# Gyeeta/gyeeta

Hardware: AMD Instinct MI355X
Metric: events/sec ingested + p50/p99 quantile error vs reference, 1→8 MI355X (higher is better)
Workload: dtype int64; 1 GPU; C3/C4: 10000 hosts x 1000 services, raw 24-B tcp_ipv4_resp_event_t stream, uniform over services, 1 window (ingest + window close) per step; service_keys_total=10000000, multi_level_windows=0, td_pend_cap=1920, td_pend_cap_is_library_default=False, exchange=none, exchange_requested=none, exchange_fallback=False

## Files before the change

### gyeeta_amd/csrc/gys_device.hpp

```cpp
#pragma once

#include <hip/hip_runtime.h>
#include <stdint.h>

#include "../../include/gysketch.h"
#include "../../include/gys_tdigest_tbl.h"

#define GYS_WAVE 64
#ifndef GYS_OPAQUE_VGPR
#define GYS_OPAQUE_VGPR(x) asm volatile("" : "+v"(x))
#endif
#ifndef GYS_DYN_LDS
#define GYS_DYN_LDS(type, name) extern __shared__ type name[]
#endif
#define GYS_SEED 0xceedfeadu
#define GYS_GOLDEN 0x9e3779b9u
#define GYS_NOSLOT 0xFFFFFFFFu
#define GYS_EMPTY_KEY 0xFFFFFFFFFFFFFFFFull

#ifndef GYS_KERNARG
#define GYS_KERNARG 1
#endif
#if GYS_KERNARG && defined(__HIP_DEVICE_COMPILE__)
#define GYS_KERNARG_REF(T, name, arg)                                                             \
// ... 61 lines not shown
	jmix(a, b, c);
	return c;
}

__host__ __device__ __forceinline__ uint32_t jhash2_4w(uint32_t k0, uint32_t k1, uint32_t k2, uint32_t k3, uint32_t initval)
{
	uint32_t a = GYS_GOLDEN + k0, b = GYS_GOLDEN + k1, c = initval + k2;
	jmix(a, b, c);
	c += 16u;
	a += k3;
	jmix(a, b, c);
	return c;
}

__host__ __device__ __forceinline__ uint32_t jhash2_u64(uint64_t key, uint32_t initval)
{
	uint32_t a = GYS_GOLDEN, b = GYS_GOLDEN, c = initval;
	c += 8;
	b += (uint32_t)(key >> 32);
	a += (uint32_t)(key & 0xFFFFFFFFu);
	jmix(a, b, c);
	return c;
}

__host__ __device__ __forceinline__ uint32_t host_tbl_hash(uint32_t netns, uint32_t port)
{
	uint32_t x = netns ^ ((port & 0xFFFFu) * 0x9E3779u);
	x ^= x >> 16;
	return x * 0x85EBCA6Bu;
}
__host__ __device__ __forceinline__ uint32_t host_tbl_hash(uint64_t key48) { return host_tbl_hash((uint32_t)(key48 >> 16), (uint32_t)(key48 & 0xFFFFu)); }
__host__ __device__ __forceinline__ uint32_t host_tbl_slot(uint32_t hk, uint32_t mask) { return (hk ^ (hk >> 13)) & mask; }
__host__ __device__ __forceinline__ uint32_t host_tbl_part(uint32_t hk, uint32_t pmask) { return (hk >> 21) & pmask; }

struct HashDef {
	int32_t nthr;
	int32_t is_fixed_diff;
	int32_t arg_bits, t_bits;
	int64_t thr[14];
	int64_t fd_min, fd_maxp1, fd_diff;
};

#define GYS_HASH_DEFS_INIT                                                                                                  \
	{                                                                                                                   \
		{13, 0, 64, 64, {1, 10, 30, 60, 100, 150, 200, 300, 450, 700, 1000, 3000, 15000}, 0, 0, 0},                      \
		{12, 0, 32, 32, {1, 10, 100, 500, 1000, 5000, 25000, 50000, 100000, 300000, 1000000, 5000000}, 0, 0, 0},      \
		{13, 0, 32, 32, {1, 10, 50, 200, 500, 1000, 3000, 6000, 10000, 15000, 25000, 60000, 150000}, 0, 0, 0},        \
		{13, 0, 32, 32, {1, 10, 25, 50, 125, 400, 1000, 3000, 6000, 10000, 25000, 40000, 65000}, 0, 0, 0},            \
		{12, 0, 32, 32, {10, 25, 50, 75, 100, 150, 300, 500, 800, 1000, 2000, 5000}, 0, 0, 0},                          \
		{10, 0, 32, 32, {5, 10, 20, 40, 60, 80, 100, 140, 200, 250}, 0, 0, 0},                                          \
		{12, 0, 32, 32, {1, 5, 10, 25, 50, 75, 100, 150, 300, 500, 1000, 3000}, 0, 0, 0},                               \
		{11, 1, 64, 32, {9, 19, 29, 39, 49, 59, 69, 79, 89, 99, 100}, 0, 101, 10},                                      \
	}

__constant__ HashDef d_hash_defs[GYS_NUM_HASH_KINDS] = GYS_HASH_DEFS_INIT;
static const HashDef h_hash_defs[GYS_NUM_HASH_KINDS] = GYS_HASH_DEFS_INIT;

__host__ __device__ inline const HashDef &hash_def(int kind)
{
#ifdef __HIP_DEVICE_COMPILE__
	return d_hash_defs[kind];
#else
	return h_hash_defs[kind];
#endif
}

// ... 286 lines not shown
```

### gyeeta_amd/csrc/gys_engine.hip

```cpp
#include <hip/hip_runtime.h>

#include <algorithm>
#include <array>
#include <atomic>
#include <chrono>
#include <cmath>
#include <cstdarg>
#include <cstdio>
#include <cstdlib>
#include <cstring>
#include <deque>
#include <map>
#include <string>
#include <thread>
#include <condition_variable>
#include <mutex>
#include <unordered_map>
#include <unordered_set>
#include <vector>

#include <dlfcn.h>
#include <rccl/rccl.h>

#include "gys_kernels.hpp"
// ... 31 lines not shown
struct MachIdHash {
	size_t operator()(const MachId &m) const
	{
		uint32_t w[4];
		memcpy(w, &m.first, 8);
		memcpy(w + 2, &m.second, 8);
		uint32_t k[6] = {w[0], w[1], w[2], w[3], 0, 0};
		return jhash2<6>(k, 4, GYS_SEED);
	}
};

inline MachId to_machid(const uint8_t id[16])
{
	MachId m;
	memcpy(&m.first, id, 8);
	memcpy(&m.second, id + 8, 8);
	return m;
}

struct ProfEntry {
	double total_ms = 0;
	uint64_t launches = 0;
	std::vector<std::pair<hipEvent_t, hipEvent_t>> pending;
};

inline uint64_t align_up(uint64_t v, uint64_t a) { return (v + a - 1) / a * a; }

struct HostListeners {
	std::vector<uint64_t> tbl;
	std::vector<uint32_t> slots;
	std::vector<uint32_t> all_slots;
	std::vector<uint64_t> keys;
	uint32_t tbl_off = 0, tbl_cap = 0, lst_off = 0;
	bool on_device = false;
	bool overflow = false;
	std::vector<HostListeners> sub;
	uint32_t sub_desc = 0;
	struct LAddr {
		uint32_t ip32 = 0;
		uint32_t ip128[4] = {0, 0, 0, 0};
		bool any = true;
	};
	struct ChainEnt {
		uint32_t slot;
		LAddr a;
	};
	std::unordered_map<uint64_t, std::vector<ChainEnt>> chain;
	std::vector<ListenerCand> cands;
	std::unordered_map<uint64_t, uint32_t> cand_first;
	uint32_t cand_off = 0, cand_cap = 0;
	bool dirty = false;
	std::unordered_map<uint64_t, uint32_t> okey;
};

#define GYS_HOST_MAX_LOCAL 2048u
#define GYS_HOST_MAX_PARTS 16u

struct ArenaLayout {
	uint64_t off_hll8, off_u32, n_u32, off_i64sum, n_i64sum, off_i64max, n_i64max, total;
	uint64_t u32_cms, u32_cluster, u32_pair, u32_misc, u32_cpair;
	uint64_t i64_cms, i64_ghist, i64_pair, i64_cpair;
};

ArenaLayout arena_layout(uint32_t max_clusters, bool conn_pair)
{
	ArenaLayout a;
// ... 414 lines not shown
void host_tbl_put(HostListeners &hl, uint64_t key48, uint32_t local)
{
	const uint32_t mask = (uint32_t)hl.tbl.size() - 1;
	uint32_t h = host_tbl_slot(host_tbl_hash(key48), mask);
	while (hl.tbl[h] != GYS_HOST_TBL_EMPTY) h = (h + 1) & mask;
	hl.tbl[h] = (key48 << 16) | (uint64_t)local;
}

inline uint32_t host_part_of(uint64_t key48, uint32_t nparts) { return host_tbl_part(host_tbl_hash(key48), nparts - 1u); }

#define GYS_HOST_TBL_SPARSE 4096u
inline uint32_t host_tbl_capacity(size_t n)
{
	static const uint32_t sparse = [] { const char *e = getenv("GYS_TBL_SPARSE"); return e ? (uint32_t)atoi(e) : GYS_HOST_TBL_SPARSE; }();
	const uint32_t c4 = next_pow2(std::max<uint64_t>(16, (uint64_t)n * 4));
	return c4 <= sparse ? c4 : std::max<uint32_t>(std::min<uint32_t>(sparse, c4), next_pow2(std::max<uint64_t>(16, (uint64_t)n * 2)));
}

int host_tbl_upload(gys_ctx *c, HostListeners &hl, uint32_t desc, uint32_t part, uint32_t nparts, uint32_t cand_off, bool *ok)
{
	*ok = true;
	if (!hl.on_device || hl.tbl.size() > hl.tbl_cap) {
		if (c->htbl_used + hl.tbl.size() > c->htbl_cap || c->hlst_used + hl.tbl.size() / 2 > c->hlst_cap) {
			*ok = false;
			return GYS_OK;
		}
		hl.tbl_off = (uint32_t)c->htbl_used;
		hl.tbl_cap = (uint32_t)hl.tbl.size();
		c->htbl_used += hl.tbl.size();
		hl.lst_off = (uint32_t)c->hlst_used;
		c->hlst_used += hl.tbl.size() / 2;
		hl.on_device = true;
	}
	HIPCHK(hipMemcpyAsync(c->htbl + hl.tbl_off, hl.tbl.data(), hl.tbl.size() * 8, hipMemcpyHostToDevice, c->stream));
	if (!hl.slots.empty()) HIPCHK(hipMemcpyAsync(c->hlst + hl.lst_off, hl.slots.data(), hl.slots.size() * 4, hipMemcpyHostToDevice, c->stream));
	const HostDesc hd{hl.tbl_off, (uint32_t)hl.tbl.size() - 1, (uint32_t)hl.slots.size(), hl.lst_off, part, nparts - 1u, cand_off, 0u};
	HIPCHK(hipMemcpyAsync(c->hdesc + desc, &hd, sizeof(hd), hipMemcpyHostToDevice, c->stream));
	HIPCHK(hipStreamSynchronize(c->stream));
	return GYS_OK;
}

int host_cands_upload(gys_ctx *c, HostListeners &hl)
{
	if (hl.cands.empty()) return GYS_OK;
	if (hl.cands.size() > hl.cand_cap) {
		const uint64_t want = std::max<uint64_t>(16, next_pow2(hl.cands.size()));
		const uint64_t bound = 4ull * c->cfg.max_services + 64ull * c->cfg.max_hosts;
		if (c->cand_used + want > bound) {
			set_err("listener candidate pool exhausted");
			return GYS_ERR_NOMEM;
		}
		if (c->cand_used + want > c->cand_cap) {
			uint64_t ncap = std::max<uint64_t>(c->cand_cap * 2, 4096);
			while (ncap < c->cand_used + want) ncap *= 2;
			ncap = std::min(ncap, bound);
			ListenerCand *np = nullptr;
			HIPCHK(hipMalloc((void **)&np, ncap * sizeof(ListenerCand)));
			if (c->cand_pool) {
				HIPCHK(hipMemcpyAsync(np, c->cand_pool, c->cand_used * sizeof(ListenerCand), hipMemcpyDeviceToDevice, c->stream));
				HIPCHK(hipStreamSynchronize(c->stream));
				HIPCHK(hipFree(c->cand_pool));
			}
			c->cand_pool = np;
			c->cand_cap = ncap;
		}
		hl.cand_off = (uint32_t)c->cand_used;
		hl.cand_cap = (uint32_t)want;
		c->cand_used += want;
	}
// ... 325 lines not shown
	const bool td = c->cfg.enable_tdigest != 0;
	if (td && n > c->cfg.max_batch_events) {
		set_err("batch of %llu events exceeds max_batch_events %llu", (unsigned long long)n, (unsigned long long)c->cfg.max_batch_events);
		return GYS_ERR_NOMEM;
	}
	if (n >= (1ull << 31)) {
		set_err("batch too large (u32 offsets)");
		return GYS_ERR_INVAL;
	}
	for (uint32_t s = 0; s < nsegs; ++s) {
		if (segs_host[s].host_slot >= c->hosts.size() || segs_host[s].first_event > n || (s && segs_host[s].first_event < segs_host[s - 1].first_event)) {
			set_err("bad resp segment %u", s);
			return GYS_ERR_INVAL;
		}
	}
	gys_ctx::SegSlot &slot = c->seg_ring[c->seg_next];
	c->seg_next = (c->seg_next + 1) % GYS_SEG_RING;
	if (!slot.done) HIPCHK(hipEventCreateWithFlags(&slot.done, hipEventDisableTiming));
	HIPCHK(hipEventSynchronize(slot.done));
	if (nsegs > slot.cap) {
		if (slot.host) HIPCHK(hipHostFree(slot.host));
		if (slot.dev) HIPCHK(hipFree(slot.dev));
		slot.host = slot.dev = nullptr;
		slot.cap = std::max<uint32_t>(nsegs, 1024);
		HIPCHK(hipHostMalloc((void **)&slot.host, (uint64_t)slot.cap * sizeof(gys_resp_seg), hipHostMallocDefault));
		HIPCHK(hipMalloc((void **)&slot.dev, (uint64_t)slot.cap * sizeof(gys_resp_seg)));
	}
	memcpy(slot.host, segs_host, (uint64_t)nsegs * sizeof(gys_resp_seg));
	for (uint32_t s = 0; s < nsegs; ++s) ((gys_resp_seg *)slot.host)[s].reserved = 0;
	HIPCHK(hipMemcpyAsync(slot.dev, slot.host, (uint64_t)nsegs * sizeof(gys_resp_seg), hipMemcpyHostToDevice, c->stream));
	const gys_resp_seg *segs_dev = slot.dev;

	bool host_local = td && c->cfg.resp_path != 1 && c->nsvc != 0, host_split = false, host_parts = false;
	uint32_t max_tbl = 16, max_l = 1;
	uint64_t max_len = 0, nwg = 0;
	bool cands = false;
	if (host_local) {
		c->batch_stamp++;
		for (uint32_t s = 0; s < nsegs && host_local; ++s) {
			const uint32_t host = segs_host[s].host_slot;
			const HostListeners &hl = c->host_lst[host];
			cands = cands || !hl.chain.empty();
			const uint64_t len = (s + 1 < nsegs ? segs_host[s + 1].first_event : n) - segs_host[s].first_event;
			if (c->host_seen[host] == c->batch_stamp || hl.overflow) host_local = false;
			c->host_seen[host] = c->batch_stamp;
			max_len = std::max(max_len, len);
			if (hl.sub.empty()) {
				if (!hl.on_device) host_local = false;
				max_tbl = std::max<uint32_t>(max_tbl, (uint32_t)hl.tbl.size());
				max_l = std::max<uint32_t>(max_l, (uint32_t)hl.slots.size());
				nwg += 1;
			} else {
				host_parts = true;
				for (const HostListeners &t : hl.sub) {
					if (!t.on_device) host_local = false;
					max_tbl = std::max<uint32_t>(max_tbl, (uint32_t)t.tbl.size());
					max_l = std::max<uint32_t>(max_l, (uint32_t)t.slots.size());
				}
				nwg += hl.sub.size();
			}
		}
		const double t_host = (double)((nwg + c->ncu - 1) / c->ncu) * (double)max_len / 0.35e9;
		const double t_split = (double)n * (double)std::max<uint64_t>(nwg, 1) / (double)std::max<uint32_t>(nsegs, 1) / 40.0e9 + 20e-6;
		if (host_local && max_len > GYS_SPLIT_PART && (c->cfg.resp_path == 3 || (c->cfg.resp_path == 0 && t_split < t_host))) host_split = true;
	}
	const int mode = v6 ? 2 : cands ? 1 : 0;
	const uint32_t nsvc = c->nsvc;
	uint32_t *cms32 = (uint32_t *)(c->arena + c->al.off_u32) + c->al.u32_cms;
	unsigned long long *ghist = (unsigned long long *)(c->arena + c->al.off_i64sum) + c->al.i64_ghist;
	long long *gmax = (long long *)(c->arena + c->al.off_i64max);
	if (td) {
		HIPCHK(hipMemsetAsync(c->merge_count, 0, 8 * 4, c->stream));
		c->resp_dirty = true;
	}
	FinP fin{};
	if (td) {
		fin.td_cur = c->td_cur;
		fin.td_meta = c->td_meta;
		fin.nsvc = c->nsvc;
		fin.pcap = c->pcap;
		fin.pend_cap = c->pend_cap;
		fin.merge_fast = c->merge_fast;
		static const bool class2_huge = getenv("GYS_CLASS2_HUGE") != nullptr || getenv("GYS_OLD_HUGE") != nullptr;
		fin.class2_max = class2_huge ? 0u : GYS_MERGE_LDS_MAX;
		fin.epoch = c->epoch;
		fin.resp_win = c->resp_win;
		fin.list[FIN_CLASS0] = c->merge_list;
		fin.list[FIN_CLASS1] = c->merge_list1;
		fin.list[FIN_CLASS2] = c->merge_list2;
// ... 67 lines not shown
			if (xbytes > slot.xcap) {
				if (slot.xhost) HIPCHK(hipHostFree(slot.xhost));
				if (slot.xdev) HIPCHK(hipFree(slot.xdev));
				slot.xhost = slot.xdev = nullptr;
				slot.xcap = std::max<uint64_t>(xbytes, 1u << 16);
				HIPCHK(hipHostMalloc((void **)&slot.xhost, slot.xcap, hipHostMallocDefault));
				HIPCHK(hipMalloc((void **)&slot.xdev, slot.xcap));
			}
			gys_resp_seg *vseg = (gys_resp_seg *)slot.xhost;
			uint64_t v = 0;
			for (uint32_t s = 0; s < nsegs; ++s) {
				const uint64_t first = segs_host[s].first_event;
				const uint64_t len = (s + 1 < nsegs ? segs_host[s + 1].first_event : n) - first;
				const HostListeners &hl = c->host_lst[segs_host[s].host_slot];
				const uint64_t step = host_split ? (uint64_t)GYS_SPLIT_PART : std::max<uint64_t>(len, 1);
				for (uint64_t q = 0; q * step < len; ++q) {
					if (hl.sub.empty()) {
						vseg[v++] = gys_resp_seg{segs_host[s].host_slot, 0u, first + q * step};
					} else {
						for (uint32_t lp = 0; lp < hl.sub.size(); ++lp)
							vseg[v++] = gys_resp_seg{segs_host[s].host_slot, c->cfg.max_hosts + hl.sub_desc + lp + 1u, first + q * step};
					}
				}
			}
			HIPCHK(hipMemcpyAsync(slot.xdev, slot.xhost, v * sizeof(gys_resp_seg), hipMemcpyHostToDevice, c->stream));
			hp.segs = (const gys_resp_seg *)slot.xdev;
			hp.nsegs = (uint32_t)v;
			hgrid = (uint32_t)v;
			if (host_split) c->n_batches_host_split++;
			else c->n_batches_host_local++;
		} else {
			c->n_batches_host_local++;
		}
		tpt12 = mode == 0 && (tpt == 12 || tpt == 0) && resp_host_lds_bytes(max_tbl, hp.lds_key_entries, 6144u) + 160u * 1024u - c->resp_dyn_max <= 80u * 1024u;
		tpt16 = !tpt12 && (mode != 0 || tpt == 16 || tpt == 32 || tpt == 0) && resp_host_lds_bytes(max_tbl, hp.lds_key_entries, 16384u) <= c->resp_dyn_max;
		tpt32 = tpt16 && tpt == 32 && !host_split;
		dyn = resp_host_lds_bytes(max_tbl, hp.lds_key_entries, tpt12 ? 6144u : tpt16 ? 16384u : 8192u);
		if (pre) {
			ProfScope ps(c, "prespill");
			PreSpillP pp{};
			pp.td_cur = c->td_cur;
			pp.td_prevm = c->td_prevm;
			pp.td_run = c->td_run;
			pp.td_run0 = c->td_run0;
			pp.td_run1 = c->td_run1;
			pp.counts = c->merge_count;
			pp.hot = c->pre_hot;
			pp.hot_rd = c->pre_seq & 1u;
			pp.svc_host = c->svc_host;
			pp.host_batch = c->host_batch;
			pp.batch_stamp = c->batch_stamp;
			pp.nsvc = nsvc;
			pp.pcap = c->pcap;
			pp.pend_cap = c->pend_cap;
			pp.resv = (unsigned long long *)(c->merge_count + 14);
			pp.run_limit = (uint32_t)std::min<uint64_t>(c->staged_cap - std::min<uint64_t>(n, c->staged_cap), 0xFFFFFFFFull);
			++c->pre_seq;
			hipLaunchKernelGGL(k_mark_hosts, dim3((nsegs + 255) / 256), dim3(256), 0, c->stream, segs_dev, nsegs, c->host_batch, c->batch_stamp);
			hipLaunchKernelGGL(k_prespill, dim3((nsvc + 255) / 256), dim3(256), 0, c->stream, pp);
		}
		{
			ProfScope ps(c, "resp_host");
			if (mode != 0) {
				if (host_split) launch_resp_host_mode<true, false>(c, mode, tpt16, hgrid, dyn, hp);
				else launch_resp_host_mode<false, false>(c, mode, tpt16, hgrid, dyn, hp);
			} else if (host_split) {
				if (tpt12) launch_resp_host<12, true, false>(c, hgrid, dyn, hp);
				else if (tpt16) launch_resp_host<16, true, false>(c, hgrid, dyn, hp);
// ... 3484 lines not shown
```

### gyeeta_amd/csrc/gys_kernels.hpp

```cpp
#pragma once

#include "gys_device.hpp"

namespace gys {

#define GYS_HUGE_VALUE_BITS 20
#define GYS_HUGE_BINS (1u << GYS_HUGE_VALUE_BITS)
#define GYS_ROW_BITS 6
#define GYS_ROW_MASK 0x3Fu
#define GYS_ROW_V6 0x20u
#define GYS_BM_WORDS 32u
#define GYS_STAGED_WORD(tresp, cli_port) ((uint64_t)(((uint32_t)(tresp) << GYS_ROW_BITS) | ((uint32_t)(cli_port) & 0x1Fu)))
#define GYS_STAGED_WORD_FAM(tresp, cli_port, v6) ((uint32_t)(((uint32_t)(tresp) << GYS_ROW_BITS) | ((v6) ? GYS_ROW_V6 : 0u) | ((uint32_t)(cli_port) & 0x1Fu)))

enum { CTR_RESP_EVENTS = 0, CTR_RESP_DROP_RANGE, CTR_RESP_DROP_NOLISTENER, CTR_CONN_EVENTS, CTR_CONN_UNKNOWN, CTR_LSTATE_RECORDS,
       CTR_LSTATE_MISSED, CTR_LSTATE_ERRORS, CTR_LSTATE_DELETED, CTR_TD_MERGES, CTR_TD_MERGE_VALUES, CTR_ACTCONN_RECORDS, CTR_ACTCONN_REMOTE_LISTEN, CTR_ACTCONN_UNKNOWN,
       CTR_CONN_NEW, CTR_CONN_CLOSED, CTR_CONN_CLOSED_NO_NOTIFY, CTR_CONN_CLI_SIDE, CTR_RESP_RUN_OVERFLOW, CTR_NUM };

__global__ void k_table_insert(DevTable t, const uint64_t *keys, uint32_t first_val, uint32_t n, uint32_t *nfail)
{
	const uint32_t i = blockIdx.x * blockDim.x + threadIdx.x;
	if (i >= n) return;
	const uint64_t key = keys[i];
	uint32_t h = get_uint64_hash(key) & t.mask;
// ... 709 lines not shown
{
	for (uint32_t i = tid; i < 256u; i += nthreads)
		s_bk[i] = resp_bucket((int64_t)(4u * i)) | (resp_bucket((int64_t)(4u * i + 1u)) << 8) | (resp_bucket((int64_t)(4u * i + 2u)) << 16) |
			  (resp_bucket((int64_t)(4u * i + 3u)) << 24);
}
__device__ __forceinline__ uint32_t resp_bucket_lut(const uint32_t *s_bk, uint32_t tresp)
{
	if (!GYS_BUCKET_LUT) return resp_bucket((int64_t)tresp);
#if GYS_BK_BYTES
	uint32_t bix = tresp & 1023u;
#if defined(__HIP_DEVICE_COMPILE__)
	asm volatile("" : "+v"(bix));
#endif
	const uint32_t lo = ((const volatile uint8_t *)s_bk)[bix];
#else
	const uint32_t lo = (s_bk[(tresp >> 2) & 255u] >> ((tresp & 3u) * 8u)) & 0xFFu;
#endif
	const uint32_t hi = 12u + (tresp > 3000u) + (tresp > 15000u);
	return tresp < 1024u ? lo : hi;
}

struct HostDesc {
	uint32_t tbl_off;
	uint32_t mask;
	uint32_t nlst;
	uint32_t lst_off;
	uint32_t part;
	uint32_t pmask;
	uint32_t cand_off;
	uint32_t pad;
};

#define GYS_HOST_TBL_EMPTY 0xFFFFFFFFFFFFFFFFull
#define GYS_EV_DROPPED 0xFFFFFFFFu
#define GYS_HOST_THREADS 1024
#define GYS_RESP_THREADS(TPT) (((TPT) == 12 || (TPT) == 32) ? 512 : 1024)
#define GYS_RESP_WAVES_PER_SIMD(TPT) ((TPT) == 32 ? 2 : 4)
#define GYS_SPLIT_PART 65536u

#ifdef GYS_RESP_TIMING
__device__ unsigned long long g_resp_timing[16];
#define GYS_TICK(i) do { const unsigned long long t_now__ = (unsigned long long)clock64(); tacc[i] += (uint32_t)(t_now__ - t_prev__); t_prev__ = t_now__; } while (0)
#else
#define GYS_TICK(i) do { } while (0)
#endif
struct RespHostP {
	const uint64_t *ev;
	uint64_t n;
	const gys_resp_seg *segs;
	uint32_t nsegs;
	const HostDesc *hdesc;
	const uint64_t *htbl;
	const uint32_t *hlst;
	const ListenerCand *cand;
	uint32_t *hll32;
	uint32_t *td_cur;
	uint32_t *td_pend;
	uint32_t pcap;
	uint32_t *td_run;
	const uint32_t *td_run1;
	long long run_delta;
	uint32_t *staged;
	const uint32_t *host_spill;
	uint32_t spill_stamp;
	uint64_t *counters;
	uint8_t *svc_hll;
	uint32_t svc_hll_p;
	unsigned long long *ghist;
	long long *gmax;
	uint32_t lds_tbl_entries;
	uint32_t lds_key_entries;
	FinP fin;
	uint32_t dbg;
};

__host__ __device__ __forceinline__ size_t resp_host_lds_bytes(uint32_t tbl_entries, uint32_t key_entries, uint32_t tile)
{
	return ((size_t)tbl_entries + 2u) * 8u + (size_t)key_entries * 24u + ((size_t)tile + 2u) * 6u;
}

#ifndef GYS_RESP_DBG
#define GYS_RESP_DBG 0
#endif
#ifndef GYS_GH_PER_WAVE
#define GYS_GH_PER_WAVE 0
#endif
#define GYS_GH_STRIDE 17u
#define GYS_HQ_CAP 512u
#define GYS_DST_BIAS 65536ull
#ifndef GYS_OPAQUE_LOADED4
#define GYS_OPAQUE_LOADED4(a) asm volatile("" : "+v"(a[0]), "+v"(a[1]), "+v"(a[2]), "+v"(a[3]))
#endif
#ifndef GYS_EV_NT
#define GYS_EV_NT 0
#endif
#ifndef GYS_EV_SADDR
#define GYS_EV_SADDR 1
#endif
#ifndef GYS_EV_X3
#define GYS_EV_X3 0
#endif
struct __attribute__((packed, aligned(4))) Ev3 {
	uint32_t x, y, z;
};
__device__ __forceinline__ uint32_t gys_swap_pair(uint32_t v)
{
#if defined(__HIP_DEVICE_COMPILE__)
	return (uint32_t)__builtin_amdgcn_update_dpp(0, (int)v, 0xB1, 0xF, 0xF, false);
#else
	return (uint32_t)__shfl_xor((int)v, 1, 64);
#endif
// ... 11 lines not shown
#ifndef GYS_RESP_KERNARG
#define GYS_RESP_KERNARG 1
#endif
#if GYS_RESP_KERNARG && defined(__HIP_DEVICE_COMPILE__)
	typedef const RespHostP __attribute__((address_space(4))) *KernargP;
	KernargP p_k = (KernargP)__builtin_amdgcn_kernarg_segment_ptr();
#define GYS_RESP_P_RELOAD() asm volatile("" : "+s"(p_k))
	const RespHostP &p = *(const RespHostP *)p_k;
#else
#define GYS_RESP_P_RELOAD() (void)0
	const RespHostP &p = p_arg;
#endif
	constexpr uint32_t T = GYS_RESP_THREADS(TPT);
	constexpr uint32_t TILE = (uint32_t)TPT * T;
	constexpr bool DBG = GYS_RESP_DBG != 0;
	constexpr bool V6 = MODE == 2;
	constexpr uint32_t SW = V6 ? GYS_EV6_WORDS : 3u;
	static_assert(MODE == 0 || TPT != 32, "the register-prefetch form exists for the plain IPv4 instance only");
	GYS_DYN_LDS(uint64_t, s_dyn);
	__shared__ uint32_t s_wsum[T / 64];
	__shared__ uint32_t s_drop[2];
	__shared__ uint32_t s_floor[2];
	__shared__ uint32_t s_fqm[4];
	__shared__ unsigned long long s_gh[16 * GYS_GH_STRIDE];
	__shared__ int32_t s_gmax;
	__shared__ uint32_t s_bk[GYS_BUCKET_LUT ? 256 : 1];
	__shared__ uint32_t s_hq[SPILL ? 1 : GYS_HQ_CAP];
	__shared__ uint32_t s_hqn;
	__shared__ FinWg s_fin;
	__shared__ uint32_t s_park[64];
	if (GYS_BUCKET_LUT && !SPILL) resp_bucket_lut_init(s_bk, threadIdx.x, T);
	const uint32_t Lc = p.lds_key_entries;
	uint64_t *s_tbl = s_dyn;
	uint64_t *s_dst = s_dyn + p.lds_tbl_entries + 2u;
	uint32_t *s_cur = (uint32_t *)(s_dst + Lc);
	uint32_t *s_slot = s_cur + Lc;
	uint32_t *s_ts2 = s_slot + Lc;
	uint32_t *s_val = s_ts2 + 2u * Lc;
	uint16_t *s_key = (uint16_t *)(s_val + TILE + 2u);
	const uint32_t tid = threadIdx.x, lane = tid & 63u, wave = tid >> 6;
	const gys_resp_seg seg = p.segs[blockIdx.x];
	const uint64_t e0 = seg.first_event;
	uint32_t nx = blockIdx.x + 1;
	if (seg.reserved)
		while (nx < p.nsegs && p.segs[nx].reserved && p.segs[nx].host_slot == seg.host_slot && p.segs[nx].first_event == e0) ++nx;
	uint64_t e1 = nx < p.nsegs ? p.segs[nx].first_event : p.n;
	if (e1 > p.n) e1 = p.n;
	if (e1 <= e0) return;
	if (SPILL && p.host_spill[seg.host_slot] != p.spill_stamp) return;
	const HostDesc hd = p.hdesc[seg.reserved ? seg.reserved - 1u : seg.host_slot];
	const uint32_t mask = hd.mask, L = hd.nlst;
	for (uint32_t i = tid; i <= mask; i += T) s_tbl[i] = p.htbl[hd.tbl_off + i];
	for (uint32_t k = tid; k < L; k += T) {
		const uint32_t slot = p.hlst[hd.lst_off + k];
		const uint32_t c = p.td_cur[slot];
		s_slot[k] = slot;
		s_cur[k] = SPILL ? (c & GYS_RESPILL_BIT) : c;
		s_ts2[k] = 0;
		s_ts2[Lc + k] = 0;
	}
	if (tid < 2) s_drop[tid] = 0;
	if (tid < 16u * GYS_GH_STRIDE) s_gh[tid] = 0;
	if (tid == 0) {
		s_hqn = 0;
		s_floor[0] = SPILL ? 0u : 0xFFFFFFFFu;
		s_floor[1] = 0xFFFFFFFFu;
		s_gmax = INT32_MIN;
		s_tbl[mask + 1u] = p.htbl[hd.tbl_off];
		s_val[TILE] = 0;
		s_key[TILE] = 0;
	}
	__syncthreads();
	if (!SPILL) {
		if (e1 - e0 >= 4096u) {
			uint32_t mn = 0xFFFFFFFFu;
			const uint4 *h4 = (const uint4 *)p.hll32;
			for (uint32_t i = tid; i < (1u << GYS_HLL_P) / 4u; i += T) {
				const uint4 v = h4[i];
				mn = min(min(mn, min(v.x, v.y)), min(v.z, v.w));
			}
			mn = wave_min_u32(mn);
			if (lane == 0) atomicMin(&s_floor[0], mn);
		} else if (tid == 0) {
			s_floor[0] = 0;
		}
		__syncthreads();
		if (tid == 0) s_floor[1] = s_floor[0];
		if (tid < 4) s_fqm[tid] = s_floor[0];
	}
	uint32_t hll_floor = 0;
	const uint32_t K = (L + T - 1) / T;
	const uint32_t klo = min(L, tid * K), khi = min(L, klo + K);
	uint32_t *const dst = SPILL ? p.staged : p.td_pend;
	uint32_t *const dstb = dst - GYS_DST_BIAS;

	uint32_t ndrop_range = 0, ndrop_nol = 0, tile_no = 0, dbg_sink = 0;
#ifdef GYS_RESP_TIMING
	uint32_t tacc[16] = {0, 0, 0, 0, 0, 0, 0, 0, 0, 0, 0, 0, 0, 0, 0, 0};
	unsigned long long t_prev__ = (unsigned long long)clock64();
#endif
#if GYS_EV_PREFETCH
// ... 146 lines not shown
				GYS_OPAQUE_LOADED4(w1);
				GYS_OPAQUE_LOADED4(w2);
				__builtin_amdgcn_wave_barrier();
				if (GYS_EV_DMA_AHEAD && g + 4 < TPT && (uint32_t)(g + 4) * T < rem) dma_issue((uint32_t)g + 4u);
			}
			GYS_OPAQUE_LOADED4(w0);
			GYS_OPAQUE_LOADED4(w1);
			GYS_OPAQUE_LOADED4(w2);
			GYS_TICK(0);
#if GYS_EV_PREFETCH && defined(__HIP_DEVICE_COMPILE__)
			if (!PF && !V6 && !SPILL) {
				const uint32_t g2 = (uint32_t)g + 4u;
				const uint64_t *nb = nullptr;
				uint32_t nlim = 0, nfirst = 0;
				if (g2 < (uint32_t)TPT && g2 * T < rem) {
					nb = tb; nlim = rem; nfirst = g2 * T;
				} else if (t0 + TILE < e1) {
					const uint64_t left2 = e1 - t0 - TILE;
					nb = tb + 3u * TILE; nlim = left2 < (uint64_t)TILE ? (uint32_t)left2 : TILE; nfirst = 0;
				}
				if (nb != nullptr && lane < 48u) {
					const uint32_t pu = lane / 12u, pl = lane - 12u * pu;
					const uint32_t ev0 = nfirst + pu * T + (tid & ~63u);
					const uint32_t byte = 24u * ev0 + 128u * pl;
					if (byte + 4u <= 24u * nlim) {
						const char *pa = (const char *)nb + byte;
						asm volatile("global_load_dword %0, %1, off" : "=v"(pf_sink) : "v"(pa) : "memory");
					}
				}
			}
#endif
			uint32_t tresp[4], local[4];
			uint64_t ea[4], eb[4];
			bool ok[4], more[4];
#pragma unroll
			for (int u = 0; u < 4; ++u) {
				const uint32_t netns = (uint32_t)w1[u];
				const uint32_t sport = (uint32_t)bswap16((uint16_t)(w1[u] >> 32));
				tresp[u] = (uint32_t)w2[u] - (uint32_t)(w2[u] >> 32);
				const bool range_ok = tresp[u] <= 1000000u;
				if (in[u] && !range_ok && hd.part == 0u) ndrop_range++;
				const uint32_t hk = host_tbl_hash(netns, sport);
				const bool mine = (hk & (hd.pmask << 21)) == (hd.part << 21);
				ok[u] = in[u] && range_ok && mine;
				const uint32_t h = host_tbl_slot(hk, mask);
				ea[u] = s_tbl[h];
				eb[u] = s_tbl[h + 1u];
			}
#pragma unroll
			for (int u = 0; u < 4; ++u) {
				const uint32_t netns = (uint32_t)w1[u], sport = (uint32_t)bswap16((uint16_t)(w1[u] >> 32));
				const uint32_t alo = (uint32_t)ea[u], ahi = (uint32_t)(ea[u] >> 32), blo = (uint32_t)eb[u], bhi = (uint32_t)(eb[u] >> 32);
#if GYS_PROBE_XOR
				const uint32_t sp16 = sport << 16, xa = alo ^ sp16, xb = blo ^ sp16;
				const bool hit_a = ahi == netns && xa < 0xFFFFu, hit_b = bhi == netns && xb < 0xFFFFu;
				uint32_t l = hit_b ? xb : GYS_NOSLOT;
				l = hit_a ? xa : l;
				local[u] = l;
				more[u] = ok[u] && !hit_a && !hit_b;
#else
				const bool hit_a = ahi == netns && (alo >> 16) == sport, hit_b = bhi == netns && (blo >> 16) == sport;
				const bool end_a = (alo & ahi) == 0xFFFFFFFFu, end_b = (blo & bhi) == 0xFFFFFFFFu;
				uint32_t l = (hit_b && !end_a) ? (blo & 0xFFFFu) : GYS_NOSLOT;
				l = hit_a ? (alo & 0xFFFFu) : l;
				local[u] = l;
				more[u] = ok[u] && !hit_a && !hit_b && !end_a && !end_b;
#endif
			}
#ifdef GYS_RESP_TIMING
			asm volatile("" : "+v"(local[0]), "+v"(local[1]), "+v"(local[2]), "+v"(local[3]));
#endif
			GYS_TICK(1);
#if GYS_PROBE_JOINT
			if (more[0] || more[1] || more[2] || more[3]) {
				uint32_t hh[4];
#pragma unroll
				for (int u = 0; u < 4; ++u)
					hh[u] = (host_tbl_slot(host_tbl_hash((uint32_t)w1[u], (uint32_t)bswap16((uint16_t)(w1[u] >> 32))), mask) + 2u) & mask;
				for (uint32_t probes = 2; probes <= mask; ++probes) {
					uint64_t e[4];
#pragma unroll
					for (int u = 0; u < 4; ++u) e[u] = s_tbl[hh[u]];
#pragma unroll
					for (int u = 0; u < 4; ++u) {
						const uint64_t key48 = ((uint64_t)(uint32_t)w1[u] << 16) | (uint64_t)bswap16((uint16_t)(w1[u] >> 32));
						const bool hit = (e[u] >> 16) == key48 && e[u] != GYS_HOST_TBL_EMPTY;
						if (more[u] && hit) local[u] = (uint32_t)(e[u] & 0xFFFFu);
						more[u] = more[u] && !hit && e[u] != GYS_HOST_TBL_EMPTY;
						hh[u] = more[u] ? ((hh[u] + 1u) & mask) : hh[u];
					}
					if (!(more[0] || more[1] || more[2] || more[3])) break;
				}
			}
#else
#pragma unroll
			for (int u = 0; u < 4; ++u) {
				if (more[u]) {
					const uint64_t key48 = ((uint64_t)(uint32_t)w1[u] << 16) | (uint64_t)bswap16((uint16_t)(w1[u] >> 32));
					uint32_t h = (host_tbl_slot(host_tbl_hash((uint32_t)(key48 >> 16), (uint32_t)(key48 & 0xFFFFu)), mask) + 2u) & mask;
					for (uint32_t probes = 2; probes <= mask; ++probes) {
						const uint64_t e = s_tbl[h];
						if ((e >> 16) == key48) {
							local[u] = (uint32_t)(e & 0xFFFFu);
							break;
						}
						if (e == GYS_HOST_TBL_EMPTY) break;
						h = (h + 1) & mask;
					}
				}
			}
#endif
#ifdef GYS_RESP_TIMING
			asm volatile("" : "+v"(local[0]), "+v"(local[1]), "+v"(local[2]), "+v"(local[3]));
#endif
			GYS_TICK(2);
			if (MODE != 0) {
#pragma unroll
				for (int u = 0; u < 4; ++u) {
					if (ok[u] && local[u] != GYS_NOSLOT && (local[u] & GYS_LOCAL_GROUP)) {
						uint32_t e32, e128[4] = {0u, 0u, 0u, 0u}, lc = 0, sl = 0;
						if (V6) {
							const uint32_t o = (uint32_t)(g + u) * T + tid;
							const uint64_t x0 = tb[GYS_EV6_WORDS * o], x1 = tb[GYS_EV6_WORDS * o + 1u];
							e128[0] = (uint32_t)x0; e128[1] = (uint32_t)(x0 >> 32); e128[2] = (uint32_t)x1; e128[3] = (uint32_t)(x1 >> 32);
							e32 = ip6_embedded_v4(e128);
						} else {
							e32 = (uint32_t)w0[u];
						}
						local[u] = cand_resolve(p.cand + hd.cand_off, local[u] & (GYS_LOCAL_GROUP - 1u), e32, e128, &lc, &sl) ? lc : GYS_NOSLOT;
					}
				}
			}
			uint32_t nwd[4], nlr[4], hidx[4], hrank[4], hcur[4], rare = 0;
// ... 3225 lines not shown
```

Before: 64.61 billion events/s.

## Rebuild per-host listener tables with seeded placement for bounded 4-slot probes

```diff
diff --git a/gyeeta_amd/csrc/gys_device.hpp b/gyeeta_amd/csrc/gys_device.hpp
--- a/gyeeta_amd/csrc/gys_device.hpp
+++ b/gyeeta_amd/csrc/gys_device.hpp
@@ -117,6 +117,10 @@
 __host__ __device__ __forceinline__ uint32_t host_tbl_hash(uint64_t key48) { return host_tbl_hash((uint32_t)(key48 >> 16), (uint32_t)(key48 & 0xFFFFu)); }
 __host__ __device__ __forceinline__ uint32_t host_tbl_slot(uint32_t hk, uint32_t mask) { return (hk ^ (hk >> 13)) & mask; }
 __host__ __device__ __forceinline__ uint32_t host_tbl_part(uint32_t hk, uint32_t pmask) { return (hk >> 21) & pmask; }
+__host__ __device__ __forceinline__ uint32_t host_tbl_slot(uint32_t hk, uint32_t mask, uint32_t seed)
+{
+	return host_tbl_slot(hk ^ ((hk >> 8) * (seed & 0xFFFFFFu)), mask);
+}
 
 struct HashDef {
 	int32_t nthr;
diff --git a/gyeeta_amd/csrc/gys_engine.hip b/gyeeta_amd/csrc/gys_engine.hip
--- a/gyeeta_amd/csrc/gys_engine.hip
+++ b/gyeeta_amd/csrc/gys_engine.hip
@@ -87,6 +87,7 @@
 	std::vector<uint32_t> all_slots;
 	std::vector<uint64_t> keys;
 	uint32_t tbl_off = 0, tbl_cap = 0, lst_off = 0;
+	uint32_t dev_entries = 0, dev_pad = 0;
 	bool on_device = false;
 	bool overflow = false;
 	std::vector<HostListeners> sub;
@@ -567,9 +568,26 @@
 		c->hlst_used += hl.tbl.size() / 2;
 		hl.on_device = true;
 	}
-	HIPCHK(hipMemcpyAsync(c->htbl + hl.tbl_off, hl.tbl.data(), hl.tbl.size() * 8, hipMemcpyHostToDevice, c->stream));
+	std::vector<uint64_t> img;
+	uint32_t pad = 0;
+	if (GYS_ONE_PROBE) {
+		std::vector<uint64_t> ents;
+		for (const uint64_t e : hl.tbl)
+			if (e != GYS_HOST_TBL_EMPTY) ents.push_back(e);
+		const uint32_t cap = next_pow2(std::max<uint64_t>(16, 2 * (uint64_t)ents.size()));
+		if (cap <= GYS_HOST_TBL_ONE_MAX && cap <= hl.tbl.size()) {
+			std::vector<uint32_t> work(3 * cap + ents.size());
+			img.resize(cap);
+			pad = host_tbl_place(ents.data(), (uint32_t)ents.size(), cap, img.data(), work.data(), hl.dev_pad);
+			if (!pad) img.clear();
+		}
+	}
+	const std::vector<uint64_t> &dev = pad ? img : hl.tbl;
+	hl.dev_entries = (uint32_t)dev.size();
+	hl.dev_pad = pad;
+	HIPCHK(hipMemcpyAsync(c->htbl + hl.tbl_off, dev.data(), dev.size() * 8, hipMemcpyHostToDevice, c->stream));
 	if (!hl.slots.empty()) HIPCHK(hipMemcpyAsync(c->hlst + hl.lst_off, hl.slots.data(), hl.slots.size() * 4, hipMemcpyHostToDevice, c->stream));
-	const HostDesc hd{hl.tbl_off, (uint32_t)hl.tbl.size() - 1, (uint32_t)hl.slots.size(), hl.lst_off, part, nparts - 1u, cand_off, 0u};
+	const HostDesc hd{hl.tbl_off, (uint32_t)dev.size() - 1, (uint32_t)hl.slots.size(), hl.lst_off, part, nparts - 1u, cand_off, pad};
 	HIPCHK(hipMemcpyAsync(c->hdesc + desc, &hd, sizeof(hd), hipMemcpyHostToDevice, c->stream));
 	HIPCHK(hipStreamSynchronize(c->stream));
 	return GYS_OK;
@@ -961,7 +979,7 @@
 	const gys_resp_seg *segs_dev = slot.dev;
 
 	bool host_local = td && c->cfg.resp_path != 1 && c->nsvc != 0, host_split = false, host_parts = false;
-	uint32_t max_tbl = 16, max_l = 1;
+	uint32_t max_tbl = 16, max_l = 1, max_form = 16;
 	uint64_t max_len = 0, nwg = 0;
 	bool cands = false;
 	if (host_local) {
@@ -976,14 +994,16 @@
 			max_len = std::max(max_len, len);
 			if (hl.sub.empty()) {
 				if (!hl.on_device) host_local = false;
-				max_tbl = std::max<uint32_t>(max_tbl, (uint32_t)hl.tbl.size());
+				max_tbl = std::max<uint32_t>(max_tbl, hl.dev_entries);
+				max_form = std::max<uint32_t>(max_form, (uint32_t)hl.tbl.size());
 				max_l = std::max<uint32_t>(max_l, (uint32_t)hl.slots.size());
 				nwg += 1;
 			} else {
 				host_parts = true;
 				for (const HostListeners &t : hl.sub) {
 					if (!t.on_device) host_local = false;
-					max_tbl = std::max<uint32_t>(max_tbl, (uint32_t)t.tbl.size());
+					max_tbl = std::max<uint32_t>(max_tbl, t.dev_entries);
+					max_form = std::max<uint32_t>(max_form, (uint32_t)t.tbl.size());
 					max_l = std::max<uint32_t>(max_l, (uint32_t)t.slots.size());
 				}
 				nwg += hl.sub.size();
@@ -1117,8 +1137,8 @@
 		} else {
 			c->n_batches_host_local++;
 		}
-		tpt12 = mode == 0 && (tpt == 12 || tpt == 0) && resp_host_lds_bytes(max_tbl, hp.lds_key_entries, 6144u) + 160u * 1024u - c->resp_dyn_max <= 80u * 1024u;
-		tpt16 = !tpt12 && (mode != 0 || tpt == 16 || tpt == 32 || tpt == 0) && resp_host_lds_bytes(max_tbl, hp.lds_key_entries, 16384u) <= c->resp_dyn_max;
+		tpt12 = mode == 0 && (tpt == 12 || tpt == 0) && resp_host_lds_bytes(max_form, hp.lds_key_entries, 6144u) + 160u * 1024u - c->resp_dyn_max <= 80u * 1024u;
+		tpt16 = !tpt12 && (mode != 0 || tpt == 16 || tpt == 32 || tpt == 0) && resp_host_lds_bytes(max_form, hp.lds_key_entries, 16384u) <= c->resp_dyn_max;
 		tpt32 = tpt16 && tpt == 32 && !host_split;
 		dyn = resp_host_lds_bytes(max_tbl, hp.lds_key_entries, tpt12 ? 6144u : tpt16 ? 16384u : 8192u);
 		if (pre) {
diff --git a/gyeeta_amd/csrc/gys_kernels.hpp b/gyeeta_amd/csrc/gys_kernels.hpp
--- a/gyeeta_amd/csrc/gys_kernels.hpp
+++ b/gyeeta_amd/csrc/gys_kernels.hpp
@@ -765,6 +765,67 @@
 };
 
 #define GYS_HOST_TBL_EMPTY 0xFFFFFFFFFFFFFFFFull
+#ifndef GYS_ONE_PROBE
+#define GYS_ONE_PROBE 1
+#endif
+#define GYS_PROBE_WIN (GYS_ONE_PROBE ? 4u : 2u)
+#define GYS_HOST_ONE_FLAG 0x80000000u
+#ifndef GYS_PROBE_STAGED
+#define GYS_PROBE_STAGED 1
+#endif
+#define GYS_HOST_TBL_ONE_MAX 2048u
+#define GYS_HOST_TBL_SEEDS 1024u
+
+__host__ __device__ __forceinline__ uint32_t host_tbl_seed(uint32_t i) { return i ? (((i * 0x9E37u + 0x3Bu) & 0xFFFFFFu) | 1u) : 0u; }
+
+inline uint32_t host_tbl_place(const uint64_t *ents, uint32_t n, uint32_t cap, uint64_t *out, uint32_t *work, uint32_t prev)
+{
+	const uint32_t mask = cap - 1u;
+	if (n >= cap) return 0u;
+	uint32_t *const cnt = work, *const first = work + cap, *const base = work + 2u * cap, *const ord = work + 3u * cap;
+	for (uint32_t t = 0; t <= GYS_HOST_TBL_SEEDS; ++t) {
+		const uint32_t seed = t == 0 ? (prev & 0xFFFFFFu) : host_tbl_seed(t - 1u);
+		if (t > 0 && seed == (prev & 0xFFFFFFu)) continue;
+		for (uint32_t s = 0; s < cap; ++s) cnt[s] = 0;
+		for (uint32_t i = 0; i < n; ++i) {
+			base[i] = host_tbl_slot(host_tbl_hash(ents[i] >> 16), mask, seed);
+			cnt[base[i]]++;
+		}
+		uint32_t back = 0, s0 = cap;
+		for (uint32_t lap = 0; lap < 2u && s0 == cap; ++lap)
+			for (uint32_t s = 0; s < cap; ++s) {
+				back += cnt[s];
+				if (lap == 1u && back == 0u) {
+					s0 = s;
+					break;
+				}
+				if (back) back--;
+			}
+		if (s0 == cap) continue;
+		uint32_t acc = 0;
+		for (uint32_t j = 1; j <= cap; ++j) {
+			const uint32_t s = (s0 + j) & mask;
+			first[s] = acc;
+			acc += cnt[s];
+		}
+		for (uint32_t i = 0; i < n; ++i) ord[first[base[i]]++] = i;
+		bool fits = true;
+		uint32_t placed = 0, avail = 0;
+		for (uint32_t j = 1; j <= cap && fits; ++j) {
+			const uint32_t s = (s0 + j) & mask;
+			avail += cnt[s];
+			if (placed < avail) {
+				const uint32_t i = ord[placed++];
+				fits = ((s - base[i]) & mask) < GYS_PROBE_WIN;
+				out[s] = ents[i];
+			} else {
+				out[s] = GYS_HOST_TBL_EMPTY;
+			}
+		}
+		if (fits) return seed | GYS_HOST_ONE_FLAG;
+	}
+	return 0u;
+}
 #define GYS_EV_DROPPED 0xFFFFFFFFu
 #define GYS_HOST_THREADS 1024
 #define GYS_RESP_THREADS(TPT) (((TPT) == 12 || (TPT) == 32) ? 512 : 1024)
@@ -809,7 +870,7 @@
 
 __host__ __device__ __forceinline__ size_t resp_host_lds_bytes(uint32_t tbl_entries, uint32_t key_entries, uint32_t tile)
 {
-	return ((size_t)tbl_entries + 2u) * 8u + (size_t)key_entries * 24u + ((size_t)tile + 2u) * 6u;
+	return ((size_t)tbl_entries + GYS_PROBE_WIN) * 8u + (size_t)key_entries * 24u + ((size_t)tile + 2u) * 6u;
 }
 
 #ifndef GYS_RESP_DBG
@@ -887,7 +948,7 @@
 	if (GYS_BUCKET_LUT && !SPILL) resp_bucket_lut_init(s_bk, threadIdx.x, T);
 	const uint32_t Lc = p.lds_key_entries;
 	uint64_t *s_tbl = s_dyn;
-	uint64_t *s_dst = s_dyn + p.lds_tbl_entries + 2u;
+	uint64_t *s_dst = s_dyn + p.lds_tbl_entries + GYS_PROBE_WIN;
 	uint32_t *s_cur = (uint32_t *)(s_dst + Lc);
 	uint32_t *s_slot = s_cur + Lc;
 	uint32_t *s_ts2 = s_slot + Lc;
@@ -905,6 +966,10 @@
 	if (SPILL && p.host_spill[seg.host_slot] != p.spill_stamp) return;
 	const HostDesc hd = p.hdesc[seg.reserved ? seg.reserved - 1u : seg.host_slot];
 	const uint32_t mask = hd.mask, L = hd.nlst;
+	constexpr bool WIN4 = GYS_ONE_PROBE && MODE == 0;
+	constexpr uint32_t PWIN = WIN4 ? 4u : 2u;
+	const uint32_t slot_seed = GYS_ONE_PROBE ? hd.pad : 0u;
+	const bool one_probe = WIN4 && (hd.pad & GYS_HOST_ONE_FLAG) != 0u;
 	for (uint32_t i = tid; i <= mask; i += T) s_tbl[i] = p.htbl[hd.tbl_off + i];
 	for (uint32_t k = tid; k < L; k += T) {
 		const uint32_t slot = p.hlst[hd.lst_off + k];
@@ -921,7 +986,11 @@
 		s_floor[0] = SPILL ? 0u : 0xFFFFFFFFu;
 		s_floor[1] = 0xFFFFFFFFu;
 		s_gmax = INT32_MIN;
+#if GYS_ONE_PROBE
+		for (uint32_t i = 0; i + 1u < GYS_PROBE_WIN; ++i) s_tbl[mask + 1u + i] = p.htbl[hd.tbl_off + (i & mask)];
+#else
 		s_tbl[mask + 1u] = p.htbl[hd.tbl_off];
+#endif
 		s_val[TILE] = 0;
 		s_key[TILE] = 0;
 	}
@@ -1134,6 +1203,16 @@
 #endif
 			uint32_t tresp[4], local[4];
 			uint64_t ea[4], eb[4];
+#if GYS_ONE_PROBE
+			uint64_t ec[4], ed[4];
+			uint32_t hs[4];
+			auto probe_ld = [&](int u) {
+				ea[u] = s_tbl[hs[u]];
+				eb[u] = s_tbl[hs[u] + 1u];
+				ec[u] = WIN4 ? s_tbl[hs[u] + 2u] : GYS_HOST_TBL_EMPTY;
+				ed[u] = WIN4 ? s_tbl[hs[u] + 3u] : GYS_HOST_TBL_EMPTY;
+			};
+#endif
 			bool ok[4], more[4];
 #pragma unroll
 			for (int u = 0; u < 4; ++u) {
@@ -1145,10 +1224,22 @@
 				const uint32_t hk = host_tbl_hash(netns, sport);
 				const bool mine = (hk & (hd.pmask << 21)) == (hd.part << 21);
 				ok[u] = in[u] && range_ok && mine;
-				const uint32_t h = host_tbl_slot(hk, mask);
+				const uint32_t h = host_tbl_slot(hk, mask, slot_seed);
+#if GYS_ONE_PROBE
+				hs[u] = h;
+#else
 				ea[u] = s_tbl[h];
 				eb[u] = s_tbl[h + 1u];
-			}
+#endif
+			}
+#if GYS_ONE_PROBE
+			probe_ld(0);
+			probe_ld(1);
+			if (!GYS_PROBE_STAGED) {
+				probe_ld(2);
+				probe_ld(3);
+			}
+#endif
 #pragma unroll
 			for (int u = 0; u < 4; ++u) {
 				const uint32_t netns = (uint32_t)w1[u], sport = (uint32_t)bswap16((uint16_t)(w1[u] >> 32));
@@ -1156,18 +1247,51 @@
 #if GYS_PROBE_XOR
 				const uint32_t sp16 = sport << 16, xa = alo ^ sp16, xb = blo ^ sp16;
 				const bool hit_a = ahi == netns && xa < 0xFFFFu, hit_b = bhi == netns && xb < 0xFFFFu;
+#if GYS_ONE_PROBE
+				const uint32_t xc = (uint32_t)ec[u] ^ sp16, xd = (uint32_t)ed[u] ^ sp16;
+				const bool hit_c = (uint32_t)(ec[u] >> 32) == netns && xc < 0xFFFFu, hit_d = (uint32_t)(ed[u] >> 32) == netns && xd < 0xFFFFu;
+				uint32_t l = hit_d ? xd : GYS_NOSLOT;
+				l = hit_c ? xc : l;
+				l = hit_b ? xb : l;
+				l = hit_a ? xa : l;
+				local[u] = l;
+				more[u] = ok[u] && !one_probe && !hit_a && !hit_b && !hit_c && !hit_d;
+#else
 				uint32_t l = hit_b ? xb : GYS_NOSLOT;
 				l = hit_a ? xa : l;
 				local[u] = l;
 				more[u] = ok[u] && !hit_a && !hit_b;
+#endif
 #else
 				const bool hit_a = ahi == netns && (alo >> 16) == sport, hit_b = bhi == netns && (blo >> 16) == sport;
 				const bool end_a = (alo & ahi) == 0xFFFFFFFFu, end_b = (blo & bhi) == 0xFFFFFFFFu;
+#if GYS_ONE_PROBE
+				const uint32_t clo = (uint32_t)ec[u], chi = (uint32_t)(ec[u] >> 32), dlo = (uint32_t)ed[u], dhi = (uint32_t)(ed[u] >> 32);
+				const bool end_c = (clo & chi) == 0xFFFFFFFFu, end_d = (dlo & dhi) == 0xFFFFFFFFu;
+				const bool hit_c = chi == netns && (clo >> 16) == sport && !end_c, hit_d = dhi == netns && (dlo >> 16) == sport && !end_d;
+				uint32_t l = hit_d ? (dlo & 0xFFFFu) : GYS_NOSLOT;
+				l = hit_c ? (clo & 0xFFFFu) : l;
+				l = (hit_b && !end_b) ? (blo & 0xFFFFu) : l;
+				l = (hit_a && !end_a) ? (alo & 0xFFFFu) : l;
+				local[u] = l;
+				more[u] = ok[u] && !one_probe && l == GYS_NOSLOT && !end_a && !end_b && (!WIN4 || (!end_c && !end_d));
+#else
 				uint32_t l = (hit_b && !end_a) ? (blo & 0xFFFFu) : GYS_NOSLOT;
 				l = hit_a ? (alo & 0xFFFFu) : l;
 				local[u] = l;
 				more[u] = ok[u] && !hit_a && !hit_b && !end_a && !end_b;
 #endif
+#endif
+#if GYS_ONE_PROBE
+				if (GYS_PROBE_STAGED && u < 2) {
+#if defined(__HIP_DEVICE_COMPILE__)
+					asm volatile("" : "+v"(local[u]) : : "memory");
+#else
+					GYS_MEM_FENCE();
+#endif
+					probe_ld(u + 2);
+				}
+#endif
 			}
 #ifdef GYS_RESP_TIMING
 			asm volatile("" : "+v"(local[0]), "+v"(local[1]), "+v"(local[2]), "+v"(local[3]));
@@ -1178,8 +1302,8 @@
 				uint32_t hh[4];
 #pragma unroll
 				for (int u = 0; u < 4; ++u)
-					hh[u] = (host_tbl_slot(host_tbl_hash((uint32_t)w1[u], (uint32_t)bswap16((uint16_t)(w1[u] >> 32))), mask) + 2u) & mask;
-				for (uint32_t probes = 2; probes <= mask; ++probes) {
+					hh[u] = (host_tbl_slot(host_tbl_hash((uint32_t)w1[u], (uint32_t)bswap16((uint16_t)(w1[u] >> 32))), mask, slot_seed) + PWIN) & mask;
+				for (uint32_t probes = PWIN; probes <= mask; ++probes) {
 					uint64_t e[4];
 #pragma unroll
 					for (int u = 0; u < 4; ++u) e[u] = s_tbl[hh[u]];
@@ -1199,8 +1323,8 @@
 			for (int u = 0; u < 4; ++u) {
 				if (more[u]) {
 					const uint64_t key48 = ((uint64_t)(uint32_t)w1[u] << 16) | (uint64_t)bswap16((uint16_t)(w1[u] >> 32));
-					uint32_t h = (host_tbl_slot(host_tbl_hash((uint32_t)(key48 >> 16), (uint32_t)(key48 & 0xFFFFu)), mask) + 2u) & mask;
-					for (uint32_t probes = 2; probes <= mask; ++probes) {
+					uint32_t h = (host_tbl_slot(host_tbl_hash((uint32_t)(key48 >> 16), (uint32_t)(key48 & 0xFFFFu)), mask, slot_seed) + PWIN) & mask;
+					for (uint32_t probes = PWIN; probes <= mask; ++probes) {
 						const uint64_t e = s_tbl[h];
 						if ((e >> 16) == key48) {
 							local[u] = (uint32_t)(e & 0xFFFFu);
```

After: 64.99 billion events/s, median of 6. No clear change (+0.6%).
